# jandevaan/zzflate

Measured on AMD Instinct MI355X. Metric: input GB/s compressed (whole node) + ratio, level 1, 1/2/4/8 MI355X, higher is better.
Workload: dtype u8; 1 GPU; 1024 MiB synthetic text per GPU (zz_generate_device kind=text, seed 0x5eed0002), level 1, zlib container, 32768-byte packets, input and output resident in HBM; level=1, packet_size=32768, bytes_per_gpu=1073741824, format=zlib, warm_window=0

## Files before the change

zzflate_amd/__init__.py:

```python
import ctypes
import enum
import os
from dataclasses import dataclass

from . import build as _build

__all__ = [
    "Format", "Config", "ZzFlateError", "ZzFlateEncode", "ZzFlateEncodeToCallback", "adler32x", "combine",
    "crc32", "crc32_combine", "bound", "Context", "lib", "DEFAULT_PACKET", "generate_host", "header", "trailer",
    "MEMBERS_BLOCK", "members_bound", "members_header", "gzi_bytes", "packet_checksums_host",
]

DEFAULT_PACKET = 32768
POINTS_SPACING = 131072
MEMBERS_BLOCK = 65280
MEMBERS_NO_EOF = 1
_ERR = (1 << 64) - 1


class Format(enum.IntEnum):
    Zlib = 0
    Gzip = 1
    Deflate = 2

# ... 78 lines not shown
        "zz_header": (i32, [i32, vp]),
        "zz_trailer": (i32, [i32, u32, u64, vp]),
        "zz_adler32": (u32, [u32, vp, u64]),
        "zz_adler32_combine": (u32, [u32, u32, u64]),
        "zz_crc32": (u32, [vp, u64, u32]),
        "zz_crc32_combine": (u32, [u32, u32, u64]),
        "zz_generate_device": (i32, [vp, i32, u64, u64, vp, u64, vp]),
        "zz_generate_host": (i32, [i32, u64, u64, vp, u64]),
        "zz_debug_reset_devices": (None, []),
        "zz_debug_host_staging_bytes": (u64, []),
        "zz_debug_lds_atomic_order": (i32, [vp, u32, pu64, pu64]),
        "zz_debug_force_lds_order": (None, [i32]),
        "zz_debug_peer_state": (i32, [i32, i32]),
        "zz_debug_last_pulls": (None, [ctypes.POINTER(i32), ctypes.POINTER(i32)]),
        "zz_debug_lds_order_verdict": (i32, [i32]),
        "zz_debug_code_lengths": (i32, [vp, u32, vp, vp, vp, vp, vp, vp]),
        "zz_last_error": (ctypes.c_char_p, []),
        "zz_version": (ctypes.c_char_p, []),
        "zz_build_flags": (ctypes.c_char_p, []),
        "zz_debug_force_lds_violation": (None, [i32]),
        "zz_debug_reset_lds_order": (None, [i32]),
        "zz_debug_l1_kernel": (i32, [vp]),
        "zz_debug_l2_kernel": (i32, [vp]),
    }
    optional = {"zz_build_flags", "zz_debug_force_lds_violation", "zz_debug_reset_lds_order", "zz_debug_l1_kernel", "zz_debug_l2_kernel"}
    for name, (res, args) in sig.items():
        if name in optional and not hasattr(L, name):
            continue
        fn = getattr(L, name)
        fn.restype = res
        fn.argtypes = args
    return L


lib = _load()
_CALLBACK = ctypes.CFUNCTYPE(ctypes.c_int, ctypes.c_void_p, ctypes.POINTER(ctypes.c_uint8), ctypes.c_uint64)


def _check(rc):
    if rc != 0:
        raise ZzFlateError(rc, lib.zz_last_error().decode())


def _cfg(config):
    return _CConfig(int(config.format), int(config.level), 1 if config.threaded else 0)


def bound(n, format=Format.Zlib, level=1, packet_size=DEFAULT_PACKET):
# ... 588 lines not shown
```

zzflate_amd/csrc/zz_api.hip:

```cpp
#include <hip/hip_runtime.h>
#include <atomic>
#include <condition_variable>
#include <mutex>
#include <string>
#include <thread>
#include <vector>
#include <algorithm>
#include <cstdio>
#include <cstdlib>
#include <cstring>

#include "../../include/zzflate_amd.h"
#include "zz_common.h"
#include "zz_wave.h"
#include "zz_checksum.h"
#include "zz_emit.h"
#include "zz_level0.h"
#include "zz_level1.h"
#include "zz_level1p.h"
#include "zz_level2.h"
#include "zz_stream2.h"
#include "zz_compact.h"
#include "zz_datagen.h"
#include "zz_verify.h"
// ... 105 lines not shown
    zz_buf<unsigned long long> d_verify;
    struct {
        zz_buf<uint32_t> first; zz_buf<uint64_t> slotbase; zz_buf<uint8_t> tails;
        zz_buf<zz_batch_desc> desc;
        zz_buf<zz_batch_totals> d_tot; zz_pin<zz_batch_totals> h_tot;
    } bat;
    struct {
        zz_buf<const uint8_t*> srcs; zz_buf<uint64_t> ns, moff; zz_buf<uint8_t> stored;
        zz_buf<zz_mw_state> d_st; zz_pin<zz_mw_state> h_st;
        uint64_t members = 0, stored_members = 0;
    } mw;
    zz_buf<uint32_t> d_work;
    zz_buf<uint64_t> d_log;
    struct {
        bool active = false; hipStream_t st = nullptr; uint32_t npk = 0; int level = 0; bool whole = false;
        bool order_checked = false;
        const uint8_t* d_src = nullptr; uint64_t n = 0, halo = 0; bool last_is_final = false; uint8_t* d_dst = nullptr; uint64_t cap = 0;
        int format = 0, cks_kind = 0, level_asked = 0; uint32_t P = 0; uint32_t warm = 0;
    } pend;
    zz_pin<uint32_t> h_err;
    uint32_t warm = 0;
    bool extended = false;
    bool timing = false;
    hipEvent_t ev0 = nullptr, ev1 = nullptr;
    bool have_time = false;
    struct {
        zz_buf<uint32_t> st;
        zz_buf<uint32_t> pend;
        zz_buf<uint32_t> pcnt, prem;
        zz_buf<uint64_t> ends; zz_buf<uint32_t> stat;
        zz_buf<uint64_t> cand;
        zz_buf<zz_cks> cks;
        zz_buf<unsigned long long> tot;
        zz_buf<zz_inf_serial_out> sres; zz_buf<uint32_t> ok;
        zz_buf<unsigned long long> items_ctr;
        zz_pin<unsigned long long> items_host;
        int last_path = 0; uint64_t last_pending = 0; uint32_t last_rounds = 0;
        zz_buf<uint8_t> stage; zz_buf<uint32_t> xcarry;
        struct { uint64_t first_packet = 0, packets = 0, pending = 0; uint32_t attempts = 0; } range;
        zz_buf<zi_read> rng_reads; zz_buf<zi_read_desc> rng_desc;
        zz_buf<zz_rng_totals> rng_tot; zz_pin<zz_rng_totals> rng_host;
        struct { uint64_t packets = 0, retried = 0; uint32_t attempts = 0, waves = 0; } ranges;
        zz_buf<zz_cks> side, scks; zz_buf<zz_cks_total> side_total; zz_buf<uint32_t> verdict;
        std::vector<uint64_t> last_index;
        struct { zz_buf<uint64_t> rows; zz_buf<zz_pt_stat> stat; zz_buf<unsigned int> next; } pts;
        struct {
// ... 45 lines not shown
    uint64_t per;
    if (level == 0) per = (uint64_t)P + 10;
    else if (level == 1) per = ((uint64_t)9 * P + 10 + 7) / 8 + 6;
    else per = (uint64_t)P + 11;
    return header_len(format) + npk * per + trailer_len(format) + 16;
}

static bool lds_order_ok(int device);
extern "C" int zz_ctx_create(int device, zz_ctx** out)
{
    if (!out) { set_err("null out"); return ZZ_E_ARG; }
    int count = 0;
    hipError_t e = hipGetDeviceCount(&count);
    if (e != hipSuccess || count == 0) {
        set_err(std::string("no HIP device available (hipGetDeviceCount: ") + hipGetErrorString(e) + ", count " +
                std::to_string(count) + "): this library has no CPU encode path");
        return ZZ_E_HIP;
    }
    if (device < 0 || device >= count) { set_err("bad device index"); return ZZ_E_ARG; }
    HIPCHK(hipSetDevice(device));
    zz_ctx* c = new zz_ctx();
    c->device = device;
    const int rc = [&]() -> int {
        if (int rc = c->d_res.grow(1)) return rc;
        if (int rc = c->d_cks_total.grow(1)) return rc;
        if (int rc = c->d_err.grow(4)) return rc;
        if (int rc = c->d_work.grow(16)) return rc;
        if (int rc = c->d_prof.grow(64)) return rc;
        if (int rc = c->d_tail.grow(128)) return rc;
        HIPCHK(hipMemset(c->d_prof, 0, 64 * sizeof(unsigned long long)));
        if (int rc = c->h_res.grow(1)) return rc;
        if (int rc = c->h_err.grow(4)) return rc;
        HIPCHK(hipEventCreate(&c->ev0));
        HIPCHK(hipEventCreate(&c->ev1));
        (void)lds_order_ok(device);
        return ZZ_OK;
    }();
    if (rc) { zz_ctx_destroy(c); return rc; }
    *out = c;
    return ZZ_OK;
}

extern "C" void zz_ctx_destroy(zz_ctx* c)
{
    if (!c) return;
    (void)hipSetDevice(c->device);
// ... 302 lines not shown
    p.order_checked = p.l1p || (warm != 0 && xdepth == 0) || (p.l2p && ZZ_L2P_XCHG);
    return p;
}
static bool take_forced_violation()
{
    int left = g_force_violation.load();
    while (left > 0 && !g_force_violation.compare_exchange_weak(left, left - 1)) {}
    return left > 0;
}
enum { ERR_RERUN = 1 };
static int read_err_word(zz_ctx* c, bool order_checked)
{
    const uint32_t e = c->h_err[0];
    if (e & 4u) {
        lds_order_revoke(c->device);
        if (!order_checked) { set_err("internal: LDS-order violation reported by a kernel that does not check it"); return ZZ_E_HIP; }
        return ERR_RERUN;
    }
    if (e & 8u) { set_err("internal: a wavefront of the level-2 kernel waited for its neighbour longer than a packet can take (zz_level2p.h, l2p_wait_ge)"); return ZZ_E_HIP; }
    if (e) { set_err("internal: packet slot overflow"); return ZZ_E_NOSPACE; }
    return ZZ_OK;
}
extern "C" int zz_debug_l1_kernel(const zz_ctx* c) { return (c && plan_launch(c, 1, 0, 0, false).l1p) ? 2 : 1; }
extern "C" int zz_debug_l2_kernel(const zz_ctx* c) { return (c && plan_launch(c, 2, 0, 0, false).l2p) ? 2 : 1; }

static void begin_encode_call(zz_ctx* c) { c->have_time = false; c->have_last = false; c->idx_empty = false; }

static void launch_cks_partials(const zz_packet_params& pp, uint32_t adler_cap, hipStream_t st)
{
    if (pp.cks_kind == ZZ_CKS_CRC) hipLaunchKernelGGL(k_crc32_packets, dim3(pp.npk < 2048 ? pp.npk : 2048), dim3(ZZ_CRC_THREADS), 0, st, pp);
    else if (pp.cks_kind == ZZ_CKS_ADLER) hipLaunchKernelGGL(k_adler_packets, dim3(pp.npk < adler_cap ? pp.npk : adler_cap), dim3(ZZ_WAVE), 0, st, pp);
}
static void launch_cks_fold(zz_ctx* c, const zz_packet_params& pp, int cks_kind, hipStream_t st)
{
    if (cks_kind != ZZ_CKS_NONE)
        hipLaunchKernelGGL(k_cks_reduce, dim3(1), dim3(ZZ_RED_THREADS), 0, st, pp.cks, pp.npk, pp.packet_size, pp.n, cks_kind, c->d_cks_total);
}

static zz_packet_params packet_params(zz_ctx* c, uint32_t npk, uint32_t P, int cks_kind, const launch_plan& plan)
{
    zz_packet_params pp = {};
    pp.packet_size = P; pp.npk = npk; pp.cks_kind = cks_kind; pp.last_is_final = 1;
    pp.slots = c->slots; pp.sizes = c->sizes; pp.cks = c->cks; pp.err = c->d_err; pp.prof = c->d_prof;
    pp.dbg_viol = plan.order_checked && take_forced_violation() ? 1 : 0;
    return pp;
}
static int launch_packet_encoders(zz_ctx* c, zz_packet_params& pp, const zz_batch_map* M, int level, int xdepth, launch_plan plan, hipStream_t st)
{
    if (c->timing) HIPCHK(hipEventRecord(c->ev0, st));
    if (pp.cks_kind == ZZ_CKS_CRC) {
        if (M) hipLaunchKernelGGL(k_crc32_packets_batch, dim3(pp.npk < 2048 ? pp.npk : 2048), dim3(ZZ_CRC_THREADS), 0, st, pp, *M);
        else launch_cks_partials(pp, 0, st);
        pp.cks_kind = ZZ_CKS_NONE;
    }
    if (level == 0) return ZZ_OK;
    if (!M) hipLaunchKernelGGL(k_fill_tail, dim3(1), dim3(128), 0, st, pp.src, pp.n, c->d_tail);
    if (level >= 2) {
        launch_level2(pp, c->l2_scratch, c->d_work, st, xdepth, plan.l2p, M);
    } else if (M) {
        if (plan.l1p) hipLaunchKernelGGL(k_encode_l1p_batch, dim3(pp.npk), dim3(ZZ_L1P_THREADS), 0, st, pp, *M);
        else hipLaunchKernelGGL(k_encode_l1_batch, dim3(pp.npk), dim3(ZZ_L1_THREADS), 0, st, pp, *M);
    } else {
        static const unsigned pad_lds = [] { const char* e = getenv("ZZFLATE_L1_PAD_LDS"); return e ? (unsigned)atoi(e) : 0u; }();
        if (pp.warm && !l1_classic()) hipLaunchKernelGGL(k_encode_l1pw, dim3(pp.npk), dim3(ZZ_L1P_THREADS), pad_lds, st, pp);
        else if (pp.warm) hipLaunchKernelGGL(k_encode_l1w, dim3(pp.npk), dim3(ZZ_L1_THREADS), pad_lds, st, pp);
        else if (!plan.l1p) hipLaunchKernelGGL(k_encode_l1, dim3(pp.npk), dim3(ZZ_L1_THREADS), pad_lds, st, pp);
        else hipLaunchKernelGGL(k_encode_l1p, dim3(pp.npk), dim3(ZZ_L1P_THREADS), pad_lds, st, pp);
    }
    return ZZ_OK;
}
static int end_packet_encoders(zz_ctx* c, int level, uint32_t npk, hipStream_t st)
{
    if (c->timing) { HIPCHK(hipEventRecord(c->ev1, st)); c->have_time = true; }
    if (level != 0) hipLaunchKernelGGL(k_scan_sizes, dim3(1), dim3(ZZ_SCAN_THREADS), 0, st, c->sizes, npk, c->offsets, c->d_res);
    return ZZ_OK;
}
static int finish_err_word(zz_ctx* c, bool order_checked, hipStream_t st)
{
    HIPCHK(hipMemcpyAsync(c->h_err, c->d_err, sizeof(uint32_t), hipMemcpyDeviceToHost, st));
    HIPCHK(hipStreamSynchronize(st));
    return read_err_word(c, order_checked);
}

static int encode_finish(zz_ctx* c, zz_result* host_res);
static int encode_common(zz_ctx* c, const uint8_t* d_src, uint64_t n, uint64_t halo, bool last_is_final,
                         uint8_t* d_dst, uint64_t cap, int format, int cks_kind, bool with_container, int level,
                         uint32_t P, hipStream_t st, zz_result* host_res, bool one_parser = false)
{
    const int level_asked = level;
    if (call_pending(c)) return ZZ_E_ARG;
    begin_encode_call(c);
    uint32_t warm = level >= 1 ? c->warm : 0;
    int xdepth = 0;
    if (level >= 4 && level <= 6 && c->extended) {
        xdepth = level == 4 ? 2 : level == 5 ? 4 : 8;
        warm = level == 4 ? 8192u : 32768u;
        level = 2;
    }
    if (level < 0 || level > 3) { set_err("level must be 0..3 (zzflate.cpp:201,230)"); return ZZ_E_LEVEL; }
    if (P == 0 || P > ZZ_MAX_PACKET_SIZE) { set_err("packet size must be 1..32768"); return ZZ_E_ARG; }
    if (!d_dst || (!d_src && n)) { set_err("null buffer"); return ZZ_E_ARG; }
    HIPCHK(hipSetDevice(c->device));
    const int hl = with_container ? header_len(format) : 0;
    const int tl = with_container ? trailer_len(format) : 0;
    if (cap < (uint64_t)hl) { set_err("destination smaller than the container header"); return ZZ_E_NOSPACE; }
    const uint64_t npk64 = (n + P - 1) / P;
    if (npk64 > 0x7FFFFFFFull) { set_err("too many packets for one call"); return ZZ_E_ARG; }
    const uint32_t npk = (uint32_t)npk64;
    const uint32_t stride = slot_stride_for(level, P);
    const launch_plan plan = plan_launch(c, level, warm, xdepth, one_parser);

    HIPCHK(hipMemsetAsync(c->d_res, 0, sizeof(zz_result), st));
    HIPCHK(hipMemsetAsync(c->d_cks_total, 0, sizeof(zz_cks_total), st));
    HIPCHK(hipMemsetAsync(c->d_err, 0, sizeof(uint32_t), st));

    if (npk == 0) {
        uint8_t blk[5]; uint32_t bl;
        if (!last_is_final) bl = 0;
        else if (level == 0) { blk[0] = 1; blk[1] = 0; blk[2] = 0; blk[3] = 0xFF; blk[4] = 0xFF; bl = 5; }
        else { blk[0] = 0x03; blk[1] = 0x00; bl = 2; }
        if ((uint64_t)hl + bl + tl > cap) { set_err("destination too small"); return ZZ_E_NOSPACE; }
        uint64_t packed = 0;
        for (uint32_t i = 0; i < bl; ++i) packed |= (uint64_t)blk[i] << (8 * i);
        hipLaunchKernelGGL(k_put_small, dim3(1), dim3(1), 0, st, d_dst + hl, packed, bl, c->d_res, (uint64_t)bl);
    } else {
        if (int rc = ensure_workspace(c, level, npk, stride, xdepth, P)) return rc;
        zz_packet_params pp = packet_params(c, npk, P, cks_kind, plan);
        pp.src = d_src; pp.n = n; pp.halo = halo; pp.last_is_final = last_is_final ? 1 : 0; pp.warm = warm; pp.slot_stride = stride; pp.tail = c->d_tail;
        if (int rc = launch_packet_encoders(c, pp, nullptr, level, xdepth, plan, st)) return rc;
        if (level == 0) {
            const uint64_t total = (uint64_t)(npk - 1) * l0_packet_bytes(P, false) +
                                   l0_packet_bytes((uint32_t)(n - (uint64_t)(npk - 1) * P), last_is_final);
            if ((uint64_t)hl + total + tl > cap) { set_err("destination too small"); return ZZ_E_NOSPACE; }
            zz_l0_params q; q.pk = pp; q.dst = d_dst + hl; q.stream_mode = 0;
            uint32_t g = npk < 16384 ? npk : 16384;
            hipLaunchKernelGGL(k_encode_l0, dim3(g), dim3(256), 0, st, q);
            hipLaunchKernelGGL(k_put_small, dim3(1), dim3(1), 0, st, (uint8_t*)nullptr, 0ull, 0u, c->d_res, total);
// ... 1177 lines not shown
    return encode_common(c, (const uint8_t*)d_src, n, halo, is_last != 0, (uint8_t*)d_dst, cap, ZZ_DEFLATE, cks_kind_for(checksum),
                         false, level, P, (hipStream_t)hip_stream, nullptr);
}
extern "C" int zz_encode_shard_finish(zz_ctx* c, uint64_t* out_len, uint32_t* cks, int checksum)
{
    if (out_len) *out_len = ~0ull;
    if (!c || !out_len) { set_err("null ctx/out_len"); return ZZ_E_ARG; }
    zz_result r;
    int rc = encode_finish(c, &r);
    if (rc) return rc;
    *out_len = r.stream_bytes;
    if (cks) *cks = checksum == ZZ_ZLIB ? ((r.cks_b << 16) | r.cks_a) : r.cks_a;
    return ZZ_OK;
}

static int encode_batch(zz_ctx* c, uint32_t nitems, const uint8_t* const* d_srcs, const uint64_t* d_ns, uint8_t* const* d_dsts,
                        const uint64_t* d_caps, uint64_t* d_out_lens, int format, int level, uint32_t P, hipStream_t st, bool one_parser)
{
    const int cks_kind = cks_kind_for(format);
    begin_encode_call(c);
    if (int rc = ensure_items(c, (uint64_t)nitems + 1)) return rc;
    if (int rc = c->bat.d_tot.grow(1)) return rc;
    if (int rc = c->bat.h_tot.grow(1)) return rc;
    HIPCHK(hipMemsetAsync(c->d_err, 0, sizeof(uint32_t), st));
    hipLaunchKernelGGL(k_batch_plan, dim3(1), dim3(ZZ_SCAN_THREADS), 0, st, d_ns, nitems, P, level, c->bat.first, c->bat.slotbase, c->bat.d_tot);
    HIPCHK(hipGetLastError());
    HIPCHK(hipMemcpyAsync(c->bat.h_tot, c->bat.d_tot, sizeof(zz_batch_totals), hipMemcpyDeviceToHost, st));
    HIPCHK(hipStreamSynchronize(st));
    const uint64_t npk64 = c->bat.h_tot->npk, slot_bytes = c->bat.h_tot->slot_bytes + 256;
    if (npk64 > 0x7FFFFFFFull) { set_err("too many packets for one call"); return ZZ_E_ARG; }
    const uint32_t npk = (uint32_t)npk64;
    const launch_plan plan = plan_launch(c, level, 0, 0, one_parser);
    if (npk) if (int rc = ensure_batch_workspace(c, level, npk, slot_bytes, P)) return rc;
    zz_batch_map M;
    M.desc = c->bat.desc; M.srcs = d_srcs; M.ns = d_ns; M.first = c->bat.first; M.tails = c->bat.tails; M.npk = npk; M.level = level;
    if (npk) {
        hipLaunchKernelGGL(k_batch_desc, dim3((npk + 255) / 256), dim3(256), 0, st, c->bat.first, nitems, npk, P, level, c->bat.slotbase, c->bat.desc);
        if (level >= 1)
            hipLaunchKernelGGL(k_batch_tails, dim3(nitems < 65536 ? nitems : 65536), dim3(128), 0, st, d_srcs, d_ns, nitems, c->bat.tails);
        zz_packet_params pp = packet_params(c, npk, P, cks_kind, plan);
        if (int rc = launch_packet_encoders(c, pp, &M, level, 0, plan, st)) return rc;
        if (level == 0) {
            zz_l0_batch_params q; q.pk = pp; q.dsts = d_dsts; q.caps = d_caps; q.format = format;
            hipLaunchKernelGGL(k_encode_l0_batch, dim3(npk < 16384 ? npk : 16384), dim3(256), 0, st, q, M);
        }
        if (int rc = end_packet_encoders(c, level, npk, st)) return rc;
    }
// ... 69 lines not shown
static int encode_members(zz_ctx* c, const uint8_t* d_src, uint64_t n, uint8_t* d_dst, uint64_t cap, uint64_t* out_len, int level,
                          uint32_t B, uint32_t P, int flags, uint64_t* d_member_offsets, hipStream_t st, bool one_parser)
{
    auto& W = c->mw;
    begin_encode_call(c);
    const uint32_t m = (uint32_t)((n + B - 1) / B), ppm = (B + P - 1) / P;
    const uint32_t last = m ? (uint32_t)(n - (uint64_t)(m - 1) * B) : 0;
    const uint32_t npk = m ? (m - 1) * ppm + (last + P - 1) / P : 0;
    const auto block_slots = [&](uint32_t len) -> uint64_t {
        const uint32_t k = (len + P - 1) / P;
        return level ? (uint64_t)(k - 1) * zz_slot_stride(level, P) + zz_slot_stride(level, len - (k - 1) * P) : 0;
    };
    const uint64_t full_slots = block_slots(B);
    const uint64_t slot_bytes = m ? (uint64_t)(m - 1) * full_slots + block_slots(last) + 256 : 0;
    const uint64_t mm = (uint64_t)m + 1;
    if (int rc = ensure_items(c, mm)) return rc;
    if (int rc = W.srcs.grow(mm)) return rc;
    if (int rc = W.ns.grow(mm)) return rc;
    if (int rc = W.moff.grow(mm)) return rc;
    if (int rc = W.stored.grow(mm)) return rc;
    if (int rc = W.d_st.grow(1)) return rc;
    if (int rc = W.h_st.grow(1)) return rc;
    if (npk) if (int rc = ensure_batch_workspace(c, level, npk, level ? slot_bytes : 0, P)) return rc;
    HIPCHK(hipMemsetAsync(c->d_err, 0, sizeof(uint32_t), st));
    const launch_plan plan = plan_launch(c, level, 0, 0, one_parser);
    zz_mw_params Q;
    Q.src = d_src; Q.n = n; Q.dst = d_dst; Q.cap = cap; Q.B = B; Q.P = P; Q.members = m; Q.ppm = ppm;
    Q.eof = (flags & ZZ_MEMBERS_NO_EOF) ? 0 : ZZ_MW_EOF; Q.level = level; Q.full_slots = full_slots;
    Q.srcs = W.srcs; Q.ns = W.ns; Q.first = c->bat.first; Q.desc = c->bat.desc;
    Q.sizes = c->sizes; Q.offsets = c->offsets; Q.cks = c->cks; Q.slots = c->slots;
    Q.moff = W.moff; Q.stored = W.stored; Q.st = W.d_st; Q.user_offsets = d_member_offsets;
    if (npk) {
        hipLaunchKernelGGL(k_mw_items, dim3((m + 1 + 255) / 256), dim3(256), 0, st, Q);
        hipLaunchKernelGGL(k_mw_desc, dim3((npk + 255) / 256), dim3(256), 0, st, Q, npk);
        zz_batch_map M;
        M.desc = c->bat.desc; M.srcs = W.srcs; M.ns = W.ns; M.first = c->bat.first; M.tails = c->bat.tails; M.npk = npk; M.level = level;
        if (level >= 1)
            hipLaunchKernelGGL(k_batch_tails, dim3(m < 65536 ? m : 65536), dim3(128), 0, st, (const uint8_t* const*)W.srcs.p, (const uint64_t*)W.ns, m,
                               (uint8_t*)c->bat.tails);
        zz_packet_params pp = packet_params(c, npk, P, ZZ_CKS_CRC, plan);
        if (int rc = launch_packet_encoders(c, pp, &M, level, 0, plan, st)) return rc;
        if (int rc = end_packet_encoders(c, level, npk, st)) return rc;
    }
    hipLaunchKernelGGL(k_mw_sizes, dim3(1), dim3(ZZ_SCAN_THREADS), 0, st, Q);
    const uint32_t per_fin = ZZ_MW_FIN_THREADS / ZZ_WAVE, gf = (m + per_fin - 1) / per_fin;
    hipLaunchKernelGGL(k_mw_finalize, dim3(gf < 65536 ? (gf ? gf : 1) : 65536), dim3(ZZ_MW_FIN_THREADS), 0, st, Q);
    if (npk && level != 0) {
// ... 1007 lines not shown
```

zzflate_amd/csrc/zz_batch.h:

```cpp
#pragma once
#include "zz_level0.h"
#include "zz_level1.h"
#include "zz_level1p.h"
#include "zz_level2.h"
#include "zz_compact.h"

namespace zz {

struct zz_batch_totals {
    uint64_t npk;
    uint64_t slot_bytes;
    uint64_t nospace;
};

__device__ __forceinline__ uint32_t batch_header_len(int format) { return format == ZZ_FMT_ZLIB ? 2 : format == ZZ_FMT_GZIP ? 10 : 0; }
__device__ __forceinline__ uint32_t batch_trailer_len(int format) { return format == ZZ_FMT_ZLIB ? 4 : format == ZZ_FMT_GZIP ? 8 : 0; }

#define ZZ_BATCH_PLAN_PER 8
__global__ __launch_bounds__(ZZ_SCAN_THREADS) void k_batch_plan(const uint64_t* ns, uint32_t nitems, uint32_t P, int level,
                                                                uint32_t* first, uint64_t* slotbase, zz_batch_totals* out)
{
    __shared__ uint64_t wc[ZZ_SCAN_THREADS / ZZ_WAVE], wb[ZZ_SCAN_THREADS / ZZ_WAVE];
    const uint32_t t = threadIdx.x, lane = t & 63, wv = t >> 6;
    const uint32_t full = level ? zz_slot_stride(level, P) : 0;
// ... 84 lines not shown
    __shared__ uint64_t red_a[4], red_c[4];
    const uint32_t hl = batch_header_len(Q.format), tl = batch_trailer_len(Q.format);
    for (uint32_t g = blockIdx.x; g < M.npk; g += gridDim.x) {
        uint32_t k;
        const zz_packet_params P = zz_packet_view(Q.pk, M, g, k);
        const uint32_t item = M.desc[g].item;
        if (hl + l0_item_bytes(P.n, P.packet_size) + tl > Q.caps[item]) continue;
        uint8_t* d = Q.dsts[item] + hl + (uint64_t)k * l0_packet_bytes(P.packet_size, false);
        l0_encode_packet(P, k, d, 0, red_a, red_c);
    }
}

__global__ __launch_bounds__(ZZ_L1_THREADS) void k_encode_l1_batch(zz_packet_params B, zz_batch_map M)
{
    __shared__ uint16_t T[ZZ_HASH_SIZE];
    __shared__ uint32_t ring_words[ZZ_RING_WORDS];
    __shared__ __attribute__((aligned(512))) uint32_t tokbuf[2 * ZZ_L1_TOKSLOT];
    uint32_t k;
    const zz_packet_params P = zz_packet_view(B, M, blockIdx.x, k);
    if (uniform(threadIdx.x >> 6) == 0) l1_packet_parser<0>(P, k, T, tokbuf);
    else l1_packet_emitter(P, k, ring_words, tokbuf);
}

__global__ __launch_bounds__(ZZ_L1P_THREADS) void k_encode_l1p_batch(zz_packet_params B, zz_batch_map M)
{
    __shared__ uint16_t T[ZZ_HASH_SIZE];
    __shared__ uint32_t ring_words[ZZ_RING_WORDS];
    __shared__ __attribute__((aligned(512))) uint32_t tokbuf[2 * ZZ_L1_TOKSLOT];
    __shared__ l1p_xch X;
    uint32_t k;
    const zz_packet_params P = zz_packet_view(B, M, blockIdx.x, k);
    const uint32_t wv = uniform(threadIdx.x >> 6);
    if (wv < 2) l1p_packet_parser<0u>(P, k, T, tokbuf, &X, wv);
    else l1p_packet_emitter<0u>(P, k, ring_words, tokbuf);
}

template <bool PP>
__global__ __launch_bounds__(PP ? ZZ_L2P_THREADS : ZZ_L2_THREADS, PP ? ZZ_L2P_WPE : 5) void k_encode_l2_batch_t(zz_l2_params Q, zz_batch_map M)
{
    l2_encode_run<0u, false, PP>(Q, M);
}

__global__ __launch_bounds__(ZZ_CRC_THREADS) void k_crc32_packets_batch(zz_packet_params B, zz_batch_map M) { crc32_packets_run(B, M); }

struct zz_batch_join {
    zz_batch_map map;
    const uint32_t* sizes;
    const uint64_t* offsets;
    const zz_cks* cks;
    const uint8_t* slots;
    uint8_t* const* dsts;
    const uint64_t* caps;
    uint64_t* out_lens;
    zz_batch_totals* totals;
    uint32_t nitems;
    uint32_t packet_size;
    int format, cks_kind, level;
// ... 100 lines not shown
```

zzflate_amd/csrc/zz_common.h:

```cpp
#pragma once
#include <hip/hip_runtime.h>
#include <stdint.h>

#define ZZ_WAVE 64
#define ZZ_HASH_BITS 13
#define ZZ_HASH_SIZE (1 << ZZ_HASH_BITS)
#define ZZ_MAX_LEN 258
#define ZZ_MAX_PACKET 32768
#define ZZ_BATCH_LEN 16384

enum { ZZ_FMT_ZLIB = 0, ZZ_FMT_GZIP = 1, ZZ_FMT_DEFLATE = 2 };
enum { ZZ_CKS_NONE = 0, ZZ_CKS_ADLER = 1, ZZ_CKS_CRC = 2 };

struct zz_cks { uint32_t a, b; };

struct zz_packet_params {
    const uint8_t* src;
    uint64_t n;
    uint64_t halo;
    uint32_t packet_size;
    uint32_t npk;
    int last_is_final;
    int cks_kind;
    uint8_t* slots;
    uint32_t slot_stride;
    uint32_t* sizes;
    zz_cks* cks;
    uint32_t* err;
    unsigned long long* prof;
    uint32_t warm;
    const uint8_t* tail;
    uint32_t dbg_viol;
};
#define ZZ_ERR_SLOT_OVERFLOW 1u
#define ZZ_ERR_LDS_ORDER 4u

__host__ __device__ inline uint32_t zz_slot_stride(int level, uint32_t len)
{
    uint64_t b;
    if (level == 0) b = (uint64_t)len + 10;
    else if (level == 1) b = ((uint64_t)9 * len + 10 + 7) / 8 + 6;
    else b = (uint64_t)len + 11;
    b += 8;
    return (uint32_t)((b + 15) & ~15ull);
}

struct zz_batch_desc {
    uint32_t item;
    uint32_t k;
    uint64_t slot;
};
struct zz_batch_map {
    const zz_batch_desc* desc;
    const uint8_t* const* srcs;
    const uint64_t* ns;
// ... 81 lines not shown
```

zzflate_amd/csrc/zz_level1p.h:

```cpp
#pragma once
#include "zz_level1.h"

namespace zz {

#define ZZ_L1P_THREADS (3 * ZZ_WAVE)
#ifndef ZZ_L1P_PRIO_W
#define ZZ_L1P_PRIO_W 3
#endif
#ifndef ZZ_L1P_PRIO_F
#define ZZ_L1P_PRIO_F 1
#endif
#ifndef ZZ_L1P_PRIO_E
#define ZZ_L1P_PRIO_E 0
#endif
#ifndef ZZ_L1P_ORDER_CHECK
#define ZZ_L1P_ORDER_CHECK 0
#endif
#ifndef ZZ_L1P_EXT32
#define ZZ_L1P_EXT32 0
#endif
#ifndef ZZ_L1P_ADLER3
#define ZZ_L1P_ADLER3 1
#endif
#ifndef ZZ_L1P_ADLER_U
#define ZZ_L1P_ADLER_U 6
#endif
#ifndef ZZ_L1P_LAZY_FLUSH
#define ZZ_L1P_LAZY_FLUSH 1
#endif
typedef __attribute__((address_space(3))) uint16_t lds_u16;

#define ZZ_L1P_NONE 64u
#define ZZ_L1P_SELF 65u
struct l1p_xch {
    uint32_t told[ZZ_WAVE + 4];
    uint8_t win[ZZ_WAVE + 4];
    uint16_t scal[ZZ_WAVE];
};



template <uint32_t BIAS>
__device__ __forceinline__ void l1p_parse(const zz_packet_params& P, const l1_pk& pk, uint16_t* T, uint32_t* tokbuf, l1p_xch* X, const uint32_t pw)
{
    const int lane = lane_id();
    const uint64_t below_me = (1ull << lane) - 1, above_me = ~((2ull << lane) - 1), self_bit = 1ull << lane;
    const uint32_t n = pk.n;
    const l1p_src SRC = l1p_make_src(P, pk.src, pk.end);
    const uint32_t NB = (n + ZZ_WAVE - 1) >> 6;
    lds_u32* const slot = (lds_u32*)tokbuf + lane + pw * ZZ_L1_TOKSLOT;
    uint64_t w = 0, w2 = 0;
    {
        const uint32_t p0 = pw * ZZ_WAVE + (uint32_t)lane;
        l1p_ld128<true>(SRC, p0 < n ? p0 : n - 1, w, w2);
    }
    ZZ_PROF_DECL
    uint32_t wmin = ZZ_WAVE;
    uint32_t mycout = 0;
    uint32_t hot_until = 0;
    if (pw == 1) l1_group_barrier();
    uint32_t xlo_next = pw ? 1u + BIAS : 0xFFFF0000u;
    for (uint32_t g = pw; g < NB; g += 2) {
        const uint32_t tag = (g + 1) << 16;
        const uint32_t xlo = xlo_next;
        xlo_next = (g << 6) + (2 * ZZ_WAVE - (ZZ_WAVE - 1)) + BIAS;
        if (mycout >= 2 * ZZ_WAVE) {
            const uint32_t p = (g << 6) + (uint32_t)lane;
            uint64_t wn = 0, wn2 = 0;
// ... 274 lines not shown
                asm volatile("s_and_saveexec_b64 %0, %1\n\tds_write_b16 %2, %3\n\ts_mov_b64 exec, %0"
                             : "=&s"(saved) : "s"(rm), "v"(taddr), "v"(told) : "memory", "scc");
            }
            if (lostmask) {
                ZZ_WAVE_SYNC();
                const uint64_t wm = ballot((myset & committed & above_me) == 0) & committed & INB;
                uint64_t saved;
                asm volatile("s_and_saveexec_b64 %0, %1\n\tds_write_b16 %2, %3\n\ts_mov_b64 exec, %0"
                             : "=&s"(saved) : "s"(wm), "v"(taddr), "v"(p + 1 + BIAS) : "memory", "scc");
            }
            ZZ_WAVE_SYNC();
            w = wn;
            w2 = wn2;
        };
        if ((g << 6) + 3 * ZZ_WAVE + 15 <= n) block(std::true_type{});
        else block(std::false_type{});
    }
    if (((NB - 1) & 1u) != pw) l1_group_barrier();
    l1_group_barrier();
    if ((ballot(wmin < (uint32_t)lane) != 0 || P.dbg_viol) && lane == 0) atomicOr(P.err, ZZ_ERR_LDS_ORDER);
    ZZ_PROF_FLUSH_W(P, pw);
}

template <uint32_t BIAS>
__device__ __forceinline__ void l1p_packet_parser(const zz_packet_params& P, uint32_t k, uint16_t* T, uint32_t* tokbuf, l1p_xch* X, uint32_t pw)
{
    const int lane = lane_id();
    const l1_pk q = l1_packet_of(P, k);
    __builtin_amdgcn_s_setprio(ZZ_L1P_PRIO_F);
    uint4* t4 = (uint4*)T + pw * (ZZ_HASH_SIZE * sizeof(uint16_t) / 32);
    for (int i = lane; i < (int)(ZZ_HASH_SIZE * sizeof(uint16_t) / 32); i += ZZ_WAVE) t4[i] = make_uint4(0, 0, 0, 0);
    if (pw == 0) X->scal[lane] = 0;
    if (pw == 0) X->told[lane] = 0;
    if (pw == 1 && lane == 0) X->win[ZZ_L1P_SELF] = (uint8_t)ZZ_L1P_SELF;
    if (!BIAS && ZZ_L1P_ADLER3 && P.cks_kind == ZZ_CKS_ADLER) {
        uint32_t A = 0;
        uint64_t C = 0;
        wave_adler_part<ZZ_L1P_ADLER_U>(q.src, q.len, pw, 3, A, C);
        const uint64_t At = wave_sum64(A), Ct = wave_sum64(C);
        if (lane == 0) { uint64_t* part = (uint64_t*)(tokbuf + ZZ_L1_TOKSLOT) + 2 * pw; part[0] = At; part[1] = Ct; }
    }
    if (BIAS) {
        l1_group_barrier();
        if (pw == 0) {
            const uint64_t before = P.halo + q.off;
            uint32_t viol = 0;
            warm_prehash<BIAS, true>(T, q.src, (int32_t)(before < P.warm ? before : P.warm), q.end, 1, (uint32_t)(((uint16_t*)tokbuf + 255) - T), viol);
            if ((ballot(viol != 0) != 0 || P.dbg_viol) && lane == 0) atomicOr(P.err, ZZ_ERR_LDS_ORDER);
        }
    }
    l1_group_barrier();
    if (q.n > 0) {
        l1p_parse<BIAS>(P, q, T, tokbuf, X, pw);
    }
}

template <uint32_t BIAS>
__device__ __forceinline__ void l1p_packet_emitter(const zz_packet_params& P, uint32_t k, uint32_t* ring_words, const uint32_t* tokbuf)
{
    const int lane = lane_id();
    const l1_pk q = l1_packet_of(P, k);
    bitring ring;
    auto append_uniform = [&](uint32_t bits, uint32_t nbits) {
        if (ZZ_L1P_LAZY_FLUSH) ring_append_lazy(ring, lane == 0 ? bits : 0u, lane == 0 ? nbits : 0u);
        else ring_append_uniform(ring, bits, nbits);
    };
    if (ZZ_L1P_PRIO_E) __builtin_amdgcn_s_setprio(ZZ_L1P_PRIO_E);
    ZZ_PROF_DECL
    ring_init(ring, ring_words, q.out);
    const bool adler3 = !BIAS && ZZ_L1P_ADLER3 && P.cks_kind == ZZ_CKS_ADLER;
    uint64_t At = 0, Ct = 0;
    if (adler3) {
        uint32_t A = 0;
        uint64_t C = 0;
        wave_adler_part<ZZ_L1P_ADLER_U>(q.src, q.len, 2, 3, A, C);
        At = wave_sum64(A); Ct = wave_sum64(C);
    }
    if (BIAS) l1_group_barrier();
    else l1_group_barrier();
    ZZ_T(2);
    if (adler3) {
        if (lane == 0) {
            const uint64_t* part = (const uint64_t*)(tokbuf + ZZ_L1_TOKSLOT);
            At += part[0] + part[2]; Ct += part[1] + part[3];
            zz_cks c;
            c.a = (uint32_t)(At % ZZ_ADLER_MOD);
            c.b = (uint32_t)(((uint64_t)q.len * At - Ct) % ZZ_ADLER_MOD);
            P.cks[k] = c;
        }
    } else if (P.cks_kind == ZZ_CKS_ADLER) {
        zz_cks c = wave_adler(q.src, q.len);
        if (lane == 0) P.cks[k] = c;
    }
    ZZ_T(3);
    if (BIAS) l1_group_barrier();
    if (q.n > 0) {
        append_uniform((q.is_final ? 1u : 0u) | (1u << 1), 3);
        const uint32_t NB = (q.n + ZZ_WAVE - 1) >> 6;
        const lds_u32* slot = (const lds_u32*)tokbuf + lane;
        l1_group_barrier();
        ZZ_T(4);
        l1_group_barrier();
        ZZ_T(5); ZZ_C(11, 1);
        for (uint32_t g = 0; g < NB; ++g) {
            ZZ_T(1); ZZ_C(10, 1);
            l1_group_barrier();
            ZZ_T(0);
            const uint32_t tok = *slot;
            slot = lds_flip_slot((lds_u32*)slot);
#ifdef ZZ_L1P_X_NOEMIT
            if (g == 0)
#endif
#if ZZ_L1P_LAZY_FLUSH
            { uint32_t bits, nb; l1_token_bits(tok, bits, nb); ring_append_lazy(ring, bits, nb); }
#else
            l1_emit_tokens(ring, nullptr, tok);
#endif
        }
        append_uniform(0, 7);
    }
    if (!q.is_final) {
        append_uniform(0, 3);
        ring_pad_to_byte(ring);
        append_uniform(0xFFFE0001u, 32);
        append_uniform(q.src[q.len - 1], 8);
    } else if (q.n == 0) {
        append_uniform(1u | (1u << 1), 3);
        append_uniform(0, 7);
    }
    const uint32_t bytes = ZZ_L1P_LAZY_FLUSH ? ring_finish_lazy(ring) : ring_finish(ring);
    if (lane == 0) {
        P.sizes[k] = bytes;
        if (bytes > P.slot_stride) atomicOr(P.err, ZZ_ERR_SLOT_OVERFLOW);
    }
    ZZ_T(6);
    ZZ_PROF_FLUSH_W(P, 2);
}

__global__ __launch_bounds__(ZZ_L1P_THREADS) void k_encode_l1p(zz_packet_params P)
{
    __shared__ uint16_t T[ZZ_HASH_SIZE];
    __shared__ uint32_t ring_words[ZZ_RING_WORDS];
    __shared__ __attribute__((aligned(512))) uint32_t tokbuf[2 * ZZ_L1_TOKSLOT];
    __shared__ l1p_xch X;
    const uint32_t k = blockIdx.x;
    const uint32_t wv = uniform(threadIdx.x >> 6);
    if (wv < 2) l1p_packet_parser<0u>(P, k, T, tokbuf, &X, wv);
    else l1p_packet_emitter<0u>(P, k, ring_words, tokbuf);
}
__global__ __launch_bounds__(ZZ_L1P_THREADS) void k_encode_l1pw(zz_packet_params P)
{
    __shared__ uint16_t T[ZZ_HASH_SIZE];
    __shared__ uint32_t ring_words[ZZ_RING_WORDS];
    __shared__ __attribute__((aligned(512))) uint32_t tokbuf[2 * ZZ_L1_TOKSLOT];
    __shared__ l1p_xch X;
    const uint32_t k = blockIdx.x;
    const uint32_t wv = uniform(threadIdx.x >> 6);
    if (wv < 2) l1p_packet_parser<32768u>(P, k, T, tokbuf, &X, wv);
    else l1p_packet_emitter<32768u>(P, k, ring_words, tokbuf);
}

}
```

Before: 145.1 GB/s.

## Convert level-1 packet encoder to persistent blocks pulling packets from an atomic counter

Adds a persistent-block variant of the level-1 parallel encoder. The grid is capped at nine blocks per compute unit, and each block draws its next packet index from a device atomic counter, with the index broadcast through LDS to the parser and emitter waves. The Adler partial sums move into the exchange struct, and launch bounds now request 7 waves per SIMD. The goal is to cut block launch and tail overhead across the roughly 32K packets, at the cost of an extra atomic and barrier per packet and possible register pressure from the occupancy hint.

```diff
diff --git a/zzflate_amd/__init__.py b/zzflate_amd/__init__.py
--- a/zzflate_amd/__init__.py
+++ b/zzflate_amd/__init__.py
@@ -124,8 +124,9 @@
         "zz_debug_reset_lds_order": (None, [i32]),
         "zz_debug_l1_kernel": (i32, [vp]),
         "zz_debug_l2_kernel": (i32, [vp]),
+        "zz_debug_set_l1_grid": (None, [vp, u32]),
     }
-    optional = {"zz_build_flags", "zz_debug_force_lds_violation", "zz_debug_reset_lds_order", "zz_debug_l1_kernel", "zz_debug_l2_kernel"}
+    optional = {"zz_build_flags", "zz_debug_force_lds_violation", "zz_debug_reset_lds_order", "zz_debug_l1_kernel", "zz_debug_l2_kernel", "zz_debug_set_l1_grid"}
     for name, (res, args) in sig.items():
         if name in optional and not hasattr(L, name):
             continue
diff --git a/zzflate_amd/csrc/zz_api.hip b/zzflate_amd/csrc/zz_api.hip
--- a/zzflate_amd/csrc/zz_api.hip
+++ b/zzflate_amd/csrc/zz_api.hip
@@ -151,6 +151,8 @@
     uint32_t warm = 0;
     bool extended = false;
     bool timing = false;
+    uint32_t cus = 0;
+    uint32_t l1_grid = 0;
     hipEvent_t ev0 = nullptr, ev1 = nullptr;
     bool have_time = false;
     struct {
@@ -242,6 +244,9 @@
     zz_ctx* c = new zz_ctx();
     c->device = device;
     const int rc = [&]() -> int {
+        hipDeviceProp_t prop;
+        HIPCHK(hipGetDeviceProperties(&prop, device));
+        c->cus = prop.multiProcessorCount > 0 ? (uint32_t)prop.multiProcessorCount : 1u;
         if (int rc = c->d_res.grow(1)) return rc;
         if (int rc = c->d_cks_total.grow(1)) return rc;
         if (int rc = c->d_err.grow(4)) return rc;
@@ -590,6 +595,7 @@
     return ZZ_OK;
 }
 extern "C" int zz_debug_l1_kernel(const zz_ctx* c) { return (c && plan_launch(c, 1, 0, 0, false).l1p) ? 2 : 1; }
+extern "C" void zz_debug_set_l1_grid(zz_ctx* c, uint32_t g) { if (c) c->l1_grid = g; }
 extern "C" int zz_debug_l2_kernel(const zz_ctx* c) { return (c && plan_launch(c, 2, 0, 0, false).l2p) ? 2 : 1; }
 
 static void begin_encode_call(zz_ctx* c) { c->have_time = false; c->have_last = false; c->idx_empty = false; }
@@ -609,9 +615,14 @@
 {
     zz_packet_params pp = {};
     pp.packet_size = P; pp.npk = npk; pp.cks_kind = cks_kind; pp.last_is_final = 1;
-    pp.slots = c->slots; pp.sizes = c->sizes; pp.cks = c->cks; pp.err = c->d_err; pp.prof = c->d_prof;
+    pp.slots = c->slots; pp.sizes = c->sizes; pp.cks = c->cks; pp.err = c->d_err; pp.work = c->d_err + 3; pp.prof = c->d_prof;
     pp.dbg_viol = plan.order_checked && take_forced_violation() ? 1 : 0;
     return pp;
+}
+static uint32_t l1p_grid(const zz_ctx* c, uint32_t npk)
+{
+    const uint32_t g = c->l1_grid ? c->l1_grid : c->cus * 9u;
+    return npk < g ? npk : g;
 }
 static int launch_packet_encoders(zz_ctx* c, zz_packet_params& pp, const zz_batch_map* M, int level, int xdepth, launch_plan plan, hipStream_t st)
 {
@@ -626,14 +637,15 @@
     if (level >= 2) {
         launch_level2(pp, c->l2_scratch, c->d_work, st, xdepth, plan.l2p, M);
     } else if (M) {
-        if (plan.l1p) hipLaunchKernelGGL(k_encode_l1p_batch, dim3(pp.npk), dim3(ZZ_L1P_THREADS), 0, st, pp, *M);
+        if (plan.l1p) hipLaunchKernelGGL(k_encode_l1p_batch, dim3(l1p_grid(c, pp.npk)), dim3(ZZ_L1P_THREADS), 0, st, pp, *M);
         else hipLaunchKernelGGL(k_encode_l1_batch, dim3(pp.npk), dim3(ZZ_L1_THREADS), 0, st, pp, *M);
     } else {
         static const unsigned pad_lds = [] { const char* e = getenv("ZZFLATE_L1_PAD_LDS"); return e ? (unsigned)atoi(e) : 0u; }();
-        if (pp.warm && !l1_classic()) hipLaunchKernelGGL(k_encode_l1pw, dim3(pp.npk), dim3(ZZ_L1P_THREADS), pad_lds, st, pp);
+        if (pp.warm && !l1_classic()) hipLaunchKernelGGL(k_encode_l1pw, dim3(l1p_grid(c, pp.npk)), dim3(ZZ_L1P_THREADS), pad_lds, st, pp);
         else if (pp.warm) hipLaunchKernelGGL(k_encode_l1w, dim3(pp.npk), dim3(ZZ_L1_THREADS), pad_lds, st, pp);
         else if (!plan.l1p) hipLaunchKernelGGL(k_encode_l1, dim3(pp.npk), dim3(ZZ_L1_THREADS), pad_lds, st, pp);
-        else hipLaunchKernelGGL(k_encode_l1p, dim3(pp.npk), dim3(ZZ_L1P_THREADS), pad_lds, st, pp);
+        else if (!c->l1_grid && pp.npk <= c->cus * 9u) hipLaunchKernelGGL(k_encode_l1p, dim3(pp.npk), dim3(ZZ_L1P_THREADS), pad_lds, st, pp);
+        else hipLaunchKernelGGL(k_encode_l1p_loop, dim3(l1p_grid(c, pp.npk)), dim3(ZZ_L1P_THREADS), pad_lds, st, pp);
     }
     return ZZ_OK;
 }
@@ -680,7 +692,7 @@
 
     HIPCHK(hipMemsetAsync(c->d_res, 0, sizeof(zz_result), st));
     HIPCHK(hipMemsetAsync(c->d_cks_total, 0, sizeof(zz_cks_total), st));
-    HIPCHK(hipMemsetAsync(c->d_err, 0, sizeof(uint32_t), st));
+    HIPCHK(hipMemsetAsync(c->d_err, 0, 4 * sizeof(uint32_t), st));
 
     if (npk == 0) {
         uint8_t blk[5]; uint32_t bl;
@@ -1904,7 +1916,7 @@
     if (int rc = ensure_items(c, (uint64_t)nitems + 1)) return rc;
     if (int rc = c->bat.d_tot.grow(1)) return rc;
     if (int rc = c->bat.h_tot.grow(1)) return rc;
-    HIPCHK(hipMemsetAsync(c->d_err, 0, sizeof(uint32_t), st));
+    HIPCHK(hipMemsetAsync(c->d_err, 0, 4 * sizeof(uint32_t), st));
     hipLaunchKernelGGL(k_batch_plan, dim3(1), dim3(ZZ_SCAN_THREADS), 0, st, d_ns, nitems, P, level, c->bat.first, c->bat.slotbase, c->bat.d_tot);
     HIPCHK(hipGetLastError());
     HIPCHK(hipMemcpyAsync(c->bat.h_tot, c->bat.d_tot, sizeof(zz_batch_totals), hipMemcpyDeviceToHost, st));
@@ -2020,7 +2032,7 @@
     if (int rc = W.d_st.grow(1)) return rc;
     if (int rc = W.h_st.grow(1)) return rc;
     if (npk) if (int rc = ensure_batch_workspace(c, level, npk, level ? slot_bytes : 0, P)) return rc;
-    HIPCHK(hipMemsetAsync(c->d_err, 0, sizeof(uint32_t), st));
+    HIPCHK(hipMemsetAsync(c->d_err, 0, 4 * sizeof(uint32_t), st));
     const launch_plan plan = plan_launch(c, level, 0, 0, one_parser);
     zz_mw_params Q;
     Q.src = d_src; Q.n = n; Q.dst = d_dst; Q.cap = cap; Q.B = B; Q.P = P; Q.members = m; Q.ppm = ppm;
diff --git a/zzflate_amd/csrc/zz_batch.h b/zzflate_amd/csrc/zz_batch.h
--- a/zzflate_amd/csrc/zz_batch.h
+++ b/zzflate_amd/csrc/zz_batch.h
@@ -130,17 +130,13 @@
     else l1_packet_emitter(P, k, ring_words, tokbuf);
 }
 
-__global__ __launch_bounds__(ZZ_L1P_THREADS) void k_encode_l1p_batch(zz_packet_params B, zz_batch_map M)
+__global__ __launch_bounds__(ZZ_L1P_THREADS, 7) void k_encode_l1p_batch(zz_packet_params B, zz_batch_map M)
 {
     __shared__ uint16_t T[ZZ_HASH_SIZE];
     __shared__ uint32_t ring_words[ZZ_RING_WORDS];
     __shared__ __attribute__((aligned(512))) uint32_t tokbuf[2 * ZZ_L1_TOKSLOT];
-    __shared__ l1p_xch X;
-    uint32_t k;
-    const zz_packet_params P = zz_packet_view(B, M, blockIdx.x, k);
-    const uint32_t wv = uniform(threadIdx.x >> 6);
-    if (wv < 2) l1p_packet_parser<0u>(P, k, T, tokbuf, &X, wv);
-    else l1p_packet_emitter<0u>(P, k, ring_words, tokbuf);
+    __shared__ l1p_xch_loop X;
+    l1p_run<0u, zz_batch_map>(T, ring_words, tokbuf, &X);
 }
 
 template <bool PP>
diff --git a/zzflate_amd/csrc/zz_common.h b/zzflate_amd/csrc/zz_common.h
--- a/zzflate_amd/csrc/zz_common.h
+++ b/zzflate_amd/csrc/zz_common.h
@@ -31,6 +31,7 @@
     uint32_t warm;
     const uint8_t* tail;
     uint32_t dbg_viol;
+    uint32_t* work;
 };
 #define ZZ_ERR_SLOT_OVERFLOW 1u
 #define ZZ_ERR_LDS_ORDER 4u
diff --git a/zzflate_amd/csrc/zz_level1p.h b/zzflate_amd/csrc/zz_level1p.h
--- a/zzflate_amd/csrc/zz_level1p.h
+++ b/zzflate_amd/csrc/zz_level1p.h
@@ -37,13 +37,18 @@
     uint8_t win[ZZ_WAVE + 4];
     uint16_t scal[ZZ_WAVE];
 };
-
-
-
-template <uint32_t BIAS>
+struct l1p_xch_loop : l1p_xch {
+    uint32_t next;
+    uint32_t part[2][3];
+};
+
+
+
+template <uint32_t BIAS, bool LOOP>
 __device__ __forceinline__ void l1p_parse(const zz_packet_params& P, const l1_pk& pk, uint16_t* T, uint32_t* tokbuf, l1p_xch* X, const uint32_t pw)
 {
-    const int lane = lane_id();
+    int lane = lane_id();
+    if (LOOP) asm volatile("" : "+v"(lane));
     const uint64_t below_me = (1ull << lane) - 1, above_me = ~((2ull << lane) - 1), self_bit = 1ull << lane;
     const uint32_t n = pk.n;
     const l1p_src SRC = l1p_make_src(P, pk.src, pk.end);
@@ -364,12 +369,14 @@
     ZZ_PROF_FLUSH_W(P, pw);
 }
 
-template <uint32_t BIAS>
-__device__ __forceinline__ void l1p_packet_parser(const zz_packet_params& P, uint32_t k, uint16_t* T, uint32_t* tokbuf, l1p_xch* X, uint32_t pw)
+template <uint32_t BIAS, bool LOOP, class XCH>
+__device__ __forceinline__ uint32_t l1p_packet_parser(const zz_packet_params& P, uint32_t k, uint16_t* T, uint32_t* tokbuf, XCH* X, uint32_t pw)
 {
     const int lane = lane_id();
     const l1_pk q = l1_packet_of(P, k);
     __builtin_amdgcn_s_setprio(ZZ_L1P_PRIO_F);
+    uint32_t drawn = 0;
+    if (LOOP && pw == 0 && lane == 0) drawn = gridDim.x + atomicAdd(P.work, 1u);
     uint4* t4 = (uint4*)T + pw * (ZZ_HASH_SIZE * sizeof(uint16_t) / 32);
     for (int i = lane; i < (int)(ZZ_HASH_SIZE * sizeof(uint16_t) / 32); i += ZZ_WAVE) t4[i] = make_uint4(0, 0, 0, 0);
     if (pw == 0) X->scal[lane] = 0;
@@ -380,8 +387,13 @@
         uint64_t C = 0;
         wave_adler_part<ZZ_L1P_ADLER_U>(q.src, q.len, pw, 3, A, C);
         const uint64_t At = wave_sum64(A), Ct = wave_sum64(C);
-        if (lane == 0) { uint64_t* part = (uint64_t*)(tokbuf + ZZ_L1_TOKSLOT) + 2 * pw; part[0] = At; part[1] = Ct; }
-    }
+        if constexpr (LOOP) {
+            if (lane == 0) { X->part[pw][0] = (uint32_t)At; X->part[pw][1] = (uint32_t)Ct; X->part[pw][2] = (uint32_t)(Ct >> 32); }
+        } else {
+            if (lane == 0) { uint64_t* part = (uint64_t*)(tokbuf + ZZ_L1_TOKSLOT) + 2 * pw; part[0] = At; part[1] = Ct; }
+        }
+    }
+    if constexpr (LOOP) { if (pw == 0 && lane == 0) X->next = drawn; }
     if (BIAS) {
         l1_group_barrier();
         if (pw == 0) {
@@ -392,13 +404,15 @@
         }
     }
     l1_group_barrier();
-    if (q.n > 0) {
-        l1p_parse<BIAS>(P, q, T, tokbuf, X, pw);
-    }
-}
-
-template <uint32_t BIAS>
-__device__ __forceinline__ void l1p_packet_emitter(const zz_packet_params& P, uint32_t k, uint32_t* ring_words, const uint32_t* tokbuf)
+    uint32_t next = ~0u;
+    if constexpr (LOOP) next = uniform(*(volatile lds_u32*)&X->next);
+    if (q.n > 0) l1p_parse<BIAS, LOOP>(P, q, T, tokbuf, X, pw);
+    else if (LOOP) l1_group_barrier();
+    return next;
+}
+
+template <uint32_t BIAS, bool LOOP, class XCH>
+__device__ __forceinline__ uint32_t l1p_packet_emitter(const zz_packet_params& P, uint32_t k, uint32_t* ring_words, const uint32_t* tokbuf, const XCH* X)
 {
     const int lane = lane_id();
     const l1_pk q = l1_packet_of(P, k);
@@ -423,8 +437,13 @@
     ZZ_T(2);
     if (adler3) {
         if (lane == 0) {
-            const uint64_t* part = (const uint64_t*)(tokbuf + ZZ_L1_TOKSLOT);
-            At += part[0] + part[2]; Ct += part[1] + part[3];
+            if constexpr (LOOP) {
+                At += (uint64_t)X->part[0][0] + X->part[1][0];
+                Ct += (((uint64_t)X->part[0][2] << 32) | X->part[0][1]) + (((uint64_t)X->part[1][2] << 32) | X->part[1][1]);
+            } else {
+                const uint64_t* part = (const uint64_t*)(tokbuf + ZZ_L1_TOKSLOT);
+                At += part[0] + part[2]; Ct += part[1] + part[3];
+            }
             zz_cks c;
             c.a = (uint32_t)(At % ZZ_ADLER_MOD);
             c.b = (uint32_t)(((uint64_t)q.len * At - Ct) % ZZ_ADLER_MOD);
@@ -436,6 +455,9 @@
     }
     ZZ_T(3);
     if (BIAS) l1_group_barrier();
+    uint32_t next = ~0u;
+    if constexpr (LOOP) next = uniform(*(volatile lds_u32*)&X->next);
+    if (LOOP && q.n == 0) l1_group_barrier();
     if (q.n > 0) {
         append_uniform((q.is_final ? 1u : 0u) | (1u << 1), 3);
         const uint32_t NB = (q.n + ZZ_WAVE - 1) >> 6;
@@ -477,6 +499,39 @@
     }
     ZZ_T(6);
     ZZ_PROF_FLUSH_W(P, 2);
+    return next;
+}
+
+template <class MAP> struct l1p_args { zz_packet_params B; MAP M; };
+template <> struct l1p_args<zz_no_batch> { zz_packet_params B; zz_no_batch M; };
+template <uint32_t BIAS, class MAP>
+__device__ __forceinline__ void l1p_run(uint16_t* T, uint32_t* ring_words, uint32_t* tokbuf, l1p_xch_loop* X)
+{
+    static_assert(alignof(zz_packet_params) == 8 && alignof(l1p_args<MAP>) == 8, "the argument segment's layout");
+    typedef const l1p_args<MAP> __attribute__((address_space(4))) args_t;
+    auto args = [&]() -> const l1p_args<MAP>& {
+        args_t* a = (args_t*)__builtin_amdgcn_kernarg_segment_ptr();
+        if (!std::is_same<MAP, zz_no_batch>::value) asm volatile("" : "+s"(a));
+        return *(const l1p_args<MAP>*)a;
+    };
+    const uint32_t wv = uniform(threadIdx.x >> 6);
+    if (wv < 2) {
+        for (uint32_t g = blockIdx.x;;) {
+            const l1p_args<MAP>& A = args();
+            if (g >= zz_batch_npk(A.B, A.M)) break;
+            uint32_t k;
+            decltype(auto) P = zz_packet_view(A.B, A.M, g, k);
+            g = l1p_packet_parser<BIAS, true>(P, k, T, tokbuf, X, wv);
+        }
+    } else {
+        for (uint32_t g = blockIdx.x;;) {
+            const l1p_args<MAP>& A = args();
+            if (g >= zz_batch_npk(A.B, A.M)) break;
+            uint32_t k;
+            decltype(auto) P = zz_packet_view(A.B, A.M, g, k);
+            g = l1p_packet_emitter<BIAS, true>(P, k, ring_words, tokbuf, X);
+        }
+    }
 }
 
 __global__ __launch_bounds__(ZZ_L1P_THREADS) void k_encode_l1p(zz_packet_params P)
@@ -487,19 +542,24 @@
     __shared__ l1p_xch X;
     const uint32_t k = blockIdx.x;
     const uint32_t wv = uniform(threadIdx.x >> 6);
-    if (wv < 2) l1p_packet_parser<0u>(P, k, T, tokbuf, &X, wv);
-    else l1p_packet_emitter<0u>(P, k, ring_words, tokbuf);
-}
-__global__ __launch_bounds__(ZZ_L1P_THREADS) void k_encode_l1pw(zz_packet_params P)
+    if (wv < 2) l1p_packet_parser<0u, false>(P, k, T, tokbuf, &X, wv);
+    else l1p_packet_emitter<0u, false>(P, k, ring_words, tokbuf, &X);
+}
+__global__ __launch_bounds__(ZZ_L1P_THREADS, 7) void k_encode_l1p_loop(zz_packet_params P)
 {
     __shared__ uint16_t T[ZZ_HASH_SIZE];
     __shared__ uint32_t ring_words[ZZ_RING_WORDS];
     __shared__ __attribute__((aligned(512))) uint32_t tokbuf[2 * ZZ_L1_TOKSLOT];
-    __shared__ l1p_xch X;
-    const uint32_t k = blockIdx.x;
-    const uint32_t wv = uniform(threadIdx.x >> 6);
-    if (wv < 2) l1p_packet_parser<32768u>(P, k, T, tokbuf, &X, wv);
-    else l1p_packet_emitter<32768u>(P, k, ring_words, tokbuf);
-}
-
-}
+    __shared__ l1p_xch_loop X;
+    l1p_run<0u, zz_no_batch>(T, ring_words, tokbuf, &X);
+}
+__global__ __launch_bounds__(ZZ_L1P_THREADS, 7) void k_encode_l1pw(zz_packet_params P)
+{
+    __shared__ uint16_t T[ZZ_HASH_SIZE];
+    __shared__ uint32_t ring_words[ZZ_RING_WORDS];
+    __shared__ __attribute__((aligned(512))) uint32_t tokbuf[2 * ZZ_L1_TOKSLOT];
+    __shared__ l1p_xch_loop X;
+    l1p_run<32768u, zz_no_batch>(T, ring_words, tokbuf, &X);
+}
+
+}
```

Result: no change. 146.5 GB/s, median of 6 (+0.9%).
